# parrot-tts/Parrot-TTS

Hardware: AMD Instinct MI355X
Metric: audio samples/sec (16 kHz; see config.note) + RTF, 256-unit batch-64 per GPU (higher is better)
Workload: dtype f32 (f16x3 split products)

## Files before the change

parrot_tts_amd/csrc/conv_consts.h:

```cpp
#pragma once
namespace parrot {
enum { PRE_NONE = 0, PRE_LRELU = 1 };
enum { ACT_NONE = 0, ACT_RELU = 1, ACT_TANH = 2 };
enum { EPI_STORE = 0, EPI_ADD = 1, EPI_ADD_DIV = 2 };

constexpr int NUM_TILE_CFGS = 7;
}
```

parrot_tts_amd/csrc/host_conv.hip:

```cpp
#include "host_common.h"

#include <algorithm>
#include <cstdio>
#include <cstring>
#include <vector>

#include "conv_split.h"
#include "conv_split16.h"
#include "conv_mfma16.h"
#include "conv_valu.h"
#include "kernels_conv.h"
#include "weight_pack.h"

using namespace parrot;
static_assert(SchBf16x6::ID == PARROT_PREC_BF16X6 && SchF16x3::ID == PARROT_PREC_F16X3 && SchBf16::ID == PARROT_PREC_BF16 && SchF16::ID == PARROT_PREC_F16,
              "weight_pack.h reads a scheme off its PARROT_PREC_* number");

static int choose_cfg(int M, int k) {
    if (M <= 16) return 6;
    if (M <= 32) return 2;
    if (M <= 64) return 1;
    return (k <= 3) ? 3 : 0;
}

// ... 5 lines not shown
    static const bool on = [] { const char* e = getenv("PARROT_MFMA16"); return !e || atoi(e) != 0; }();
    return on;
}
static int small_tiles_mode() {
    static const int m = [] { const char* e = getenv("PARROT_SMALL_TILES"); return e ? atoi(e) : 2; }();
    return m;
}

int parrot::conv_build(parrot_conv** out, const parrot_conv_desc* d, int groups, const float* w, const float* bias, bool allow16) {
    if (!out || !d || !w) return fail(PARROT_E_INVALID, "conv_create: null argument");
    if (d->c_in <= 0 || d->c_out <= 0 || d->k <= 0 || d->dilation <= 0 || groups <= 0 || d->c_in % groups || d->c_out % groups)
        return fail(PARROT_E_INVALID, "conv_create: bad dimensions");
    std::unique_ptr<parrot_conv> c(new parrot_conv());
    c->d = *d;
    c->groups = groups;
    c->Cout = d->c_out;
    c->Cin = d->c_in / groups;
    int dmin = 0;
    if (d->transposed) {
        if (d->stride > 64) return fail(PARROT_E_UNSUPPORTED, "conv_create: transposed stride > 64");
        if (groups != 1 || d->dilation != 1 || d->stride <= 0) return fail(PARROT_E_UNSUPPORTED, "conv_create: transposed conv needs groups=1, dilation=1");
        const int u = d->stride, p = d->padding, k = d->k;
        int dlo = 1 << 30, dhi = -(1 << 30);
        for (int r = 0; r < u; ++r)
            for (int kap = 0; kap < k; ++kap)
                if ((r + p - kap) % u == 0) {
                    int dl = (r + p - kap) / u;
                    dlo = std::min(dlo, dl);
                    dhi = std::max(dhi, dl);
                }
        if (dlo > dhi) return fail(PARROT_E_INVALID, "conv_create: transposed conv has no taps");
        dmin = dlo;
        c->u = u;
        c->kk = dhi - dlo + 1;
        c->dil = 1;
        c->pad_left = -dlo;
        c->M = d->c_out * u;
    } else {
        if (d->stride > 1) return fail(PARROT_E_UNSUPPORTED, "conv_create: strided Conv1d is not on the path");
        c->u = 1;
        c->kk = d->k;
        c->dil = d->dilation;
        c->pad_left = d->padding;
        c->M = d->c_out;
    }
    c->Mg = c->M / groups;
    if ((c->kk - 1) * c->dil > CONV_HALO) return fail(PARROT_E_UNSUPPORTED, "conv_create: (k-1)*dilation exceeds the LDS halo (64)");
    c->cfg = (d->tile_cfg >= 0) ? d->tile_cfg : choose_cfg(c->Mg, c->kk);
    if (c->cfg >= NUM_TILE_CFGS) return fail(PARROT_E_INVALID, "conv_create: tile_cfg out of range");
    if (c->cfg == 6 && (d->transposed || groups != 1 || c->M > 16)) {
        if (d->tile_cfg == 6) return fail(PARROT_E_UNSUPPORTED, "conv_create: the 16-row tile needs a plain conv with <= 16 output channels");
        c->cfg = 2;
    }
    const TileCfg t = tile_cfg(c->cfg);
    if (groups > 1 && c->Mg % t.bm) return fail(PARROT_E_UNSUPPORTED, "conv_create: rows per group must be a multiple of the tile height");
    const int CI = t.ci, QN = CI / 8;
    c->nchunks = (c->Cin + CI - 1) / CI;
    c->n_it = c->cfg == 6 ? c->nchunks * c->kk : c->nchunks * c->kk * QN;
    const int kk = c->kk;
    const GemmWeights W{w, c->M, c->Cin, d->k, d->transposed != 0, d->c_out, c->u, d->padding, dmin};
    const int want_prec = (d->precision >= 0) ? d->precision : create_prec();
    if (want_prec > PARROT_PREC_F16) return fail(PARROT_E_INVALID, "conv_create: unknown precision");
    const bool slope_ok = d->pre_act != PRE_LRELU || (d->pre_slope >= 0.f && d->pre_slope <= 1.f);
    if (want_prec >= 1 && c->Mg >= 32 && d->tile_cfg < 0 && c->Cin % 16 == 0 && slope_ok) {
        c->prec = want_prec;
        c->cfg = (c->Mg <= 32) ? 2 : (c->Mg <= 64) ? 1 : 0;
        const TileCfg t16 = tile_cfg(c->cfg);
        if (groups > 1 && c->Mg % t16.bm) return fail(PARROT_E_UNSUPPORTED, "conv_create: rows per group must be a multiple of the tile height");
        if (scheme_is_f16(want_prec)) c->wscale = f16_weight_scale(w, (size_t)d->c_in / groups * d->c_out * d->k);
        c->mfma16 = allow16 && mfma16_enabled() && split16_has(want_prec, c->kk) && !d->transposed && groups == 1 && c->Cin % 32 == 0 && c->M >= 64;
        int rows = 32, bm = t16.bm;
        if (c->mfma16) {
            int bn16;
            rows = 16;
            split16_tile(c->M >= 128 ? 0 : 1, bm, bn16);
        }
        const int chans = 512 / rows;
        c->nchunks = (c->Cin + chans - 1) / chans;
        c->n_it16 = c->nchunks * c->kk;
        const size_t n_steps = (size_t)((c->M + bm - 1) / bm * (bm / rows)) * c->n_it16;
        const size_t n16 = (n_steps + 1) * scheme_pieces(want_prec) * 512;
        if (n16 * sizeof(uint16_t) >= ((size_t)1 << 31)) return fail(PARROT_E_UNSUPPORTED, "conv_create: packed weight stream larger than 2 GiB");
        std::vector<uint16_t> pk16(n16, 0);
        const int n_it16 = c->n_it16;
        pack_pieces(pk16.data(), n_steps, want_prec, c->wscale, W, [=](size_t st, int lane, int e) {
            const int mt = (int)(st / n_it16), ch = (int)(st % n_it16) / kk, j = (int)(st % n_it16) % kk;
            return WeightAt{mt * rows + lane % rows, ch * chans + 8 * (lane / rows) + e, j};
        });
        HIP_TRY(hipMalloc((void**)&c->wfrag16, pk16.size() * sizeof(uint16_t)));
        HIP_TRY(hipMemcpy(c->wfrag16, pk16.data(), pk16.size() * sizeof(uint16_t), hipMemcpyHostToDevice));
    } else {
        const size_t n_steps = c->cfg == 6 ? (size_t)c->n_it : (size_t)((c->M + t.bm - 1) / t.bm * (t.bm / 32)) * c->n_it;
        std::vector<float> pk((n_steps + 1) * 256, 0.f);
        if (c->cfg == 6)
            pack_f32(pk.data(), n_steps, W, [=](size_t st, int lane, int e) { return WeightAt{lane & 15, (int)st / kk * 16 + 4 * e + (lane >> 4), (int)st % kk}; });
        else {
            const int n_it = c->n_it;
            pack_f32(pk.data(), n_steps, W, [=](size_t st, int lane, int e) {
                const int mt = (int)(st / n_it), r = (int)(st % n_it), q = r % QN, j = r / QN % kk, ch = r / QN / kk;
                return WeightAt{mt * 32 + (lane & 31), ch * CI + 8 * q + 2 * e + (lane >> 5), j};
            });
        }
        HIP_TRY(hipMalloc((void**)&c->wfrag, pk.size() * sizeof(float)));
        HIP_TRY(hipMemcpy(c->wfrag, pk.data(), pk.size() * sizeof(float), hipMemcpyHostToDevice));
    }
    if (d->tile_cfg < 0 && groups == 1 && slope_ok && d->dilation == 1 && valu_kernels_enabled()) {
        if (!d->transposed && d->c_out == 1 && ((d->k == 7 && d->padding == 3) || (d->k == 1 && d->padding == 0)) &&
            (d->act == ACT_NONE || d->act == ACT_TANH))
            c->valu_kind = 1;
        if (d->transposed && d->c_out == 16 && d->k == 4 && d->stride == 2 && d->padding == 1 && d->act == ACT_NONE) c->valu_kind = 2;
        if (c->valu_kind) {
            const size_t n = (size_t)d->c_in * d->c_out * d->k;
            HIP_TRY(hipMalloc((void**)&c->wraw, n * sizeof(float)));
            HIP_TRY(hipMemcpy(c->wraw, w, n * sizeof(float), hipMemcpyHostToDevice));
        }
    }
    if (bias) {
        HIP_TRY(hipMalloc((void**)&c->bias, (size_t)d->c_out * sizeof(float)));
        HIP_TRY(hipMemcpy(c->bias, bias, (size_t)d->c_out * sizeof(float), hipMemcpyHostToDevice));
    }
    *out = c.release();
    return PARROT_OK;
}

int parrot::conv_launch(const parrot_conv* c, const float* x, const float* res, float* y, int B, int Tin, int epi, float div, hipStream_t s,
                        const ConvOpts& o) {
    const PlaneArgs& pl = o.planes;
    if (B <= 0 || Tin <= 0) return fail(PARROT_E_INVALID, "conv_run: empty batch or sequence");
    const int Tout = c->out_len(Tin);
    if (Tout <= 0) return fail(PARROT_E_INVALID, "conv_run: sequence shorter than the kernel");
    if (c->valu_kind && !res && epi == EPI_STORE && (double)c->d.c_in * Tin * 4.0 < 2147483648.0) {
        ConvValuParams q{};
        q.x = x; q.w = c->wraw; q.bias = c->bias; q.y = y;
        q.B = B; q.Cin = c->d.c_in; q.Tin = Tin; q.Tout = Tout;
        q.slope = c->d.pre_act == PRE_LRELU ? c->d.pre_slope : 1.f;
        q.act = c->d.act;
        q.row_len = o.rows.len; q.row_len_mul = o.rows.mul; q.row_len_add = o.rows.add;
        q.err = c->err_flag;
        ProfRec rec{};
        const double macs = (double)B * c->d.c_out * c->d.c_in * c->d.k * (c->d.transposed ? (double)Tin : (double)Tout);
        if (prof_on()) TRY(prof_open(rec, c->valu_kind == 1 ? PROF_VALU_CONV1 : PROF_VALU_CONVT, 2.0 * macs, 4.0 * B * ((double)c->d.c_in * Tin + (double)c->d.c_out * Tout), s));
        if (c->valu_kind == 1 && c->d.k == 7 && (Tin & 3) == 0 && (reinterpret_cast<size_t>(x) & 15) == 0 && (reinterpret_cast<size_t>(y) & 15) == 0)
            hipLaunchKernelGGL(conv1_valu7_vec_kernel, dim3((Tout + 1023) / 1024, B), dim3(256), 0, s, q);
        else if (c->valu_kind == 1 && c->d.k == 7) hipLaunchKernelGGL(conv1_valu_kernel<7>, dim3((Tout + 1023) / 1024, B), dim3(256), 0, s, q);
        else if (c->valu_kind == 1) hipLaunchKernelGGL(linear1_valu_kernel, dim3((Tout + 63) / 64, B), dim3(256), 0, s, q);
        else hipLaunchKernelGGL((convt_valu_kernel<16, 4, 2, 1>), dim3((Tin + 255) / 256, B), dim3(256), 0, s, q);
        HIP_TRY(hipGetLastError());
        if (prof_on()) TRY(prof_close(rec, s));
        return PARROT_OK;
    }
    ConvParams p{};
    p.x = x; p.wfrag = c->wfrag; p.bias = c->bias; p.res = res; p.y = y;
    p.B = B; p.Cin = c->Cin; p.Tin = Tin; p.M = c->M; p.Cout = c->Cout;
    p.Ncols = (c->u > 1) ? (Tout + c->u - 1) / c->u : Tout;
    p.Tout = Tout;
    p.k = c->kk; p.dil = c->dil; p.pad_left = c->pad_left;
    p.nchunks = c->nchunks; p.n_it = c->n_it;
    p.pre = c->d.pre_act; p.pre_slope = c->d.pre_slope; p.act = c->d.act;
    p.epi = epi; p.div = div; p.u = c->u; p.u_inv16 = (65536 + c->u - 1) / c->u;
    p.groups = c->groups; p.Mg = c->Mg;
    p.row_len = o.rows.len; p.row_len_mul = o.rows.mul; p.row_len_add = o.rows.add;
    p.acc_scale = p.out_scale = 1.f;
    p.lean = 1;
    p.n_cus = num_cus();
    p.fold_res = c->late_res ? 0 : 1;
    if (pl.xplane || pl.yplane) {
        if (!plane_ok(c) || (pl.yplane && epi != EPI_STORE)) return fail(PARROT_E_INVALID, "conv_run: operand planes need a conv_split16 layer (k = 7 / 11) and EPI_STORE");
        p.xplane = pl.xplane; p.yplane = pl.yplane;
        p.xplane_bstride = (long)plane_row_bytes(c->prec, c->Cin, Tin);
        p.yplane_bstride = (long)plane_row_bytes(c->prec, c->M, Tout);
        p.yplane_slope = pl.yslope; p.plane_only = pl.plane_only;
// ... 108 lines not shown
```

parrot_tts_amd/csrc/parrot_hip.hip:

```cpp
#include "host_common.h"

#include <algorithm>
#include <cstring>
#include <mutex>
#include <vector>

#include "conv_split.h"
#include "conv_split16.h"
#include "kernels_voc.h"
#include "resblock_split.h"
#include "resblock_fused.h"
#include "weight_pack.h"

using namespace parrot;

struct parrot_voc {
    parrot_voc_cfg cfg{};
    float* dict = nullptr;
    float* spkr = nullptr;
    DevFlag err;
    std::unique_ptr<parrot_conv> conv_pre, conv_post;
    std::vector<std::unique_ptr<parrot_conv>> ups, rb;
    std::vector<uint16_t*> rb_stream;
    std::vector<float> rb_wsc;
// ... 95 lines not shown
    const int per_rb = v->per_rb();
    if (w->n_rb != cfg->n_stages * cfg->n_kernels * per_rb) return fail(PARROT_E_INVALID, "voc_create: wrong number of resblock convs");
    query_device();
    v->scheme = create_prec();
    v->fused = create_fused();
    for (int i = 0; i < cfg->n_stages; ++i) HIP_TRY(hipEventCreateWithFlags(&v->ev_stage[i], hipEventDisableTiming));
    {
        const char* e = getenv("PARROT_PLANES");
        v->planes = e ? atoi(e) != 0 : (v->scheme == PARROT_PREC_BF16 || v->scheme == PARROT_PREC_F16);
    }
    {
        const char* e = getenv("PARROT_MRF_STREAMS");
        const bool on = e ? atoi(e) > 1 : true;
        v->mrf_auto = (e == nullptr);
        v->mrf_streams = (on && cfg->n_kernels > 1) ? cfg->n_kernels : 1;
        if (v->mrf_streams > 1) {
            for (int j = 1; j < v->mrf_streams; ++j) HIP_TRY(hipStreamCreateWithFlags(&v->ss.side[j], hipStreamNonBlocking));
            HIP_TRY(hipEventCreateWithFlags(&v->ss.ev_fork, hipEventDisableTiming));
            for (int j = 0; j < v->mrf_streams; ++j) HIP_TRY(hipEventCreateWithFlags(&v->ss.ev_last[j], hipEventDisableTiming));
        }
        for (int l = 1; l < parrot_voc::MAX_LANES; ++l) {
            HIP_TRY(hipStreamCreateWithFlags(&v->lane_stream[l], hipStreamNonBlocking));
            HIP_TRY(hipEventCreateWithFlags(&v->ev_lane_join[l], hipEventDisableTiming));
        }
        HIP_TRY(hipEventCreateWithFlags(&v->ev_lane_fork, hipEventDisableTiming));
    }
    for (int i = 0; i < cfg->n_stages; ++i) {
        const int u = cfg->upsample_rates[i], k = cfg->upsample_kernel_sizes[i];
        if (u <= 0 || k < u) return fail(PARROT_E_UNSUPPORTED, "voc_create: upsample_kernel_size must be >= upsample_rate (negative padding)");
        if ((k - u) & 1) v->odd_stage = true;
    }
    TRY(upload(&v->dict, w->dict, (size_t)cfg->num_embeddings * cfg->embedding_dim));
    if (cfg->multispkr) {
        if (!w->spkr) return fail(PARROT_E_INVALID, "voc_create: multispkr without spkr table");
        TRY(upload(&v->spkr, w->spkr, (size_t)cfg->n_spkr * cfg->embedding_dim));
    }
    TRY(v->err.init());
    const int C0 = cfg->upsample_initial_channel;
    TRY(make_conv(v->conv_pre, cfg->model_in_dim, C0, 7, 1, 3, 0, 1, PRE_NONE, 0.f, ACT_NONE, w->conv_pre_w, w->conv_pre_b));
    v->ups.resize(cfg->n_stages);
    v->rb.resize(w->n_rb);
    for (int i = 0; i < cfg->n_stages; ++i) {
        const int cin = C0 >> i, cout = C0 >> (i + 1), u = cfg->upsample_rates[i], k = cfg->upsample_kernel_sizes[i];
        v->up_total *= u;
        TRY(make_conv(v->ups[i], cin, cout, k, 1, (k - u) / 2, 1, u, PRE_LRELU, 0.1f, ACT_NONE, w->ups_w[i], w->ups_b[i]));
        for (int j = 0; j < cfg->n_kernels; ++j) {
            const int rk = cfg->resblock_kernel_sizes[j];
            const bool a16 = !(v->fused != 0 && cfg->resblock_type == 1 && resblock_split_has(cout, rk) && per_rb <= RBS_MAX_CONVS);
            for (int m = 0; m < cfg->n_dil; ++m) {
                const int dl = cfg->resblock_dilation_sizes[j][m];
                const int base = v->rb_base(i, j);
                if (cfg->resblock_type == 1) {
                    TRY(make_conv(v->rb[base + 2 * m], cout, cout, rk, dl, (rk * dl - dl) / 2, 0, 1, PRE_LRELU, 0.1f, ACT_NONE,
                                  w->rb_w[base + 2 * m], w->rb_b[base + 2 * m], 1, a16));
                    TRY(make_conv(v->rb[base + 2 * m + 1], cout, cout, rk, 1, (rk - 1) / 2, 0, 1, PRE_LRELU, 0.1f, ACT_NONE,
                                  w->rb_w[base + 2 * m + 1], w->rb_b[base + 2 * m + 1], 1, a16));
                } else {
                    TRY(make_conv(v->rb[base + m], cout, cout, rk, dl, (rk * dl - dl) / 2, 0, 1, PRE_LRELU, 0.1f, ACT_NONE,
                                  w->rb_w[base + m], w->rb_b[base + m], 1, a16));
                }
            }
        }
    }
    v->rb_stream.assign((size_t)cfg->n_stages * cfg->n_kernels, nullptr);
    v->rb_wsc.assign((size_t)w->n_rb, 1.f);
    v->rb_conv_halves.assign((size_t)cfg->n_stages * cfg->n_kernels, 0);
    const int NP = scheme_pieces(v->scheme);
    for (int i = 0; i < cfg->n_stages && v->scheme >= 1; ++i)
        for (int j = 0; j < cfg->n_kernels; ++j) {
            const int rk = cfg->resblock_kernel_sizes[j], C = v->chan(i);
            if (cfg->resblock_type != 1 || !resblock_split_has(C, rk) || per_rb > RBS_MAX_CONVS) continue;
            const int base = v->rb_base(i, j);
            const int steps = resblock_split_steps(C, rk);
            const size_t step_b = (size_t)NP * 1024, conv_b = (size_t)steps * step_b;
            v->rb_conv_halves[v->branch(i, j)] = conv_b / 2;
            if (C >= 32) {
                bool ok = true;
                for (int q = 0; q < per_rb; ++q) {
                    const parrot_conv* pc = v->rb[base + q].get();
                    ok = ok && pc->prec == v->scheme && !pc->mfma16 && pc->wfrag16 && pc->nchunks == C / 16 && (C / 32) * pc->n_it16 == steps && pc->M == C &&
                         C % tile_cfg(pc->cfg).bm == 0;
                }
                if (!ok) continue;
                uint16_t* st = nullptr;
                HIP_TRY(hipMalloc((void**)&st, (per_rb + 1) * conv_b));
                v->rb_stream[v->branch(i, j)] = st;
                for (int q = 0; q <= per_rb; ++q)
                    HIP_TRY(hipMemcpy(reinterpret_cast<char*>(st) + q * conv_b, v->rb[base + (q < per_rb ? q : 0)]->wfrag16, conv_b, hipMemcpyDeviceToDevice));
                for (int q = 0; q < per_rb; ++q) v->rb_wsc[base + q] = v->rb[base + q]->wscale;
            } else {
                const size_t step_h = (size_t)NP * 512;
                std::vector<uint16_t> pk(((size_t)per_rb * steps + 2) * step_h, 0);
                for (int q = 0; q < per_rb; ++q) {
                    const GemmWeights W{w->rb_w[base + q], 16, 16, rk, false, 0, 1, 0, 0};
                    const float wsc = scheme_is_f16(v->scheme) ? f16_weight_scale(W.w, (size_t)16 * 16 * rk) : 1.f;
                    v->rb_wsc[base + q] = wsc;
                    pack_pieces(pk.data() + (size_t)q * steps * step_h, steps, v->scheme, wsc, W, [](size_t st, int lane, int e) {
                        return WeightAt{lane & 15, 8 * ((lane >> 4) & 1) + e, 2 * (int)st + (lane >> 5)};
                    });
                }
                uint16_t* st = nullptr;
                HIP_TRY(hipMalloc((void**)&st, pk.size() * sizeof(uint16_t)));
                v->rb_stream[v->branch(i, j)] = st;
                HIP_TRY(hipMemcpy(st, pk.data(), pk.size() * sizeof(uint16_t), hipMemcpyHostToDevice));
            }
        }
    v->mrf_ok.assign((size_t)cfg->n_stages, 0);
    {
        static const bool want = [] { const char* e = getenv("PARROT_MRF_FUSED"); return !e || atoi(e) != 0; }();
        for (int i = 0; i < cfg->n_stages && want && v->fused != 0 && v->scheme >= 1 && resblock_mrf_scheme(v->scheme); ++i) {
            const int C = v->chan(i);
            if (cfg->resblock_type != 1 || !resblock_mrf_has(C) || per_rb > RBS_MAX_CONVS || cfg->n_kernels > RBS_MAX_BRANCH) continue;
            bool ok = true;
            for (int j = 0; j < cfg->n_kernels; ++j) ok = ok && (cfg->resblock_kernel_sizes[j] & 1) && v->branch_stream(i, j);
            v->mrf_ok[i] = ok && rbs_mrf_window(C) - 2 * v->stage_reach(i) >= rbs_mrf_window(C) / 2;
        }
    }
    TRY(make_conv(v->conv_post, C0 >> cfg->n_stages, 1, 7, 1, 3, 0, 1, PRE_LRELU, 0.01f, ACT_TANH, w->conv_post_w, w->conv_post_b));
    v->conv_post->err_flag = v->err;
    *out = v.release();
    return PARROT_OK;
}
extern "C" int parrot_voc_create(parrot_voc_t** out, const parrot_voc_cfg* cfg, const parrot_voc_weights* w) { return voc_create(out, cfg, w, -1, -1); }
extern "C" int parrot_voc_create_ex(parrot_voc_t** out, const parrot_voc_cfg* cfg, const parrot_voc_weights* w, int32_t precision,
                                    int32_t fused_resblocks) {
    if (precision > PARROT_PREC_F16 || fused_resblocks > 2) return fail(PARROT_E_INVALID, "voc_create_ex: precision in -1 .. 4, fused_resblocks in -1 .. 2");
    return voc_create(out, cfg, w, precision, fused_resblocks);
}
extern "C" void parrot_voc_destroy(parrot_voc_t* v) { delete v; }
extern "C" int parrot_voc_precision(const parrot_voc_t* v) { return v ? v->scheme : PARROT_E_INVALID; }
extern "C" int parrot_voc_debug_absmax(parrot_voc_t* v, float* dst_dev) {
    if (!v) return fail(PARROT_E_INVALID, "voc_debug_absmax: null handle");
    v->dbg_absmax = dst_dev;
    return PARROT_OK;
}

static size_t voc_max_act(const parrot_voc* v, int B, int U) {
    size_t mx = (size_t)B * v->cfg.upsample_initial_channel * U;
    int T = U;
    for (int i = 0; i < v->cfg.n_stages; ++i) {
        T = v->ups[i]->out_len(T);
        mx = std::max(mx, (size_t)B * v->chan(i) * (size_t)T);
    }
    return mx;
}
static long voc_out_len(const parrot_voc* v, int U) {
    long T = U;
    for (int i = 0; i < v->cfg.n_stages; ++i) T = v->ups[i]->out_len((int)T);
    return T;
}
extern "C" int64_t parrot_voc_out_len(const parrot_voc_t* v, int32_t U) { return (v && U > 0) ? voc_out_len(v, U) : 0; }

static bool resblock_fusable(const parrot_voc* v, int stage, int j) {
    const parrot_voc_cfg& c = v->cfg;
    const int C = v->chan(stage), k = c.resblock_kernel_sizes[j];
    const int fm = v->fused;
    if (fm == 0 || !(C == 16 || (C == 32 && fm == 1)) || !(k & 1)) return false;
    const int per_rb = v->per_rb(), base = v->rb_base(stage, j);
    if (per_rb > RB_MAX_CONVS) return false;
    for (int m = 0; m < c.n_dil; ++m)
        if ((k - 1) / 2 * c.resblock_dilation_sizes[j][m] > RB_PAD) return false;
    for (int q = 0; q < per_rb; ++q)
        if (v->rb[base + q]->prec != 0 || v->rb[base + q]->cfg != (C == 16 ? 6 : 2) || !v->rb[base + q]->wfrag) return false;
    return resblock_window(C) - 2 * v->branch_reach(stage, j) >= 128;
}
struct Branch {
    const float* x;
    float* y;
    float *mid, *res_a, *res_b;
    int B, T, epi;
    float div;
// ... 566 lines not shown
```

parrot_tts_amd/csrc/resblock_split.h:

```cpp
#pragma once
#include "conv_split.h"

namespace parrot {

constexpr int RBS_MAX_CONVS = 8;
constexpr int RBS_MAX_BRANCH = 4;
constexpr int RBS_MAX_ALL = RBS_MAX_CONVS * RBS_MAX_BRANCH;

#ifdef RBS_TRACE
constexpr int RBS_TRACE_STAMPS = 128;
__device__ unsigned long long g_rbs_trace[8 * RBS_TRACE_STAMPS];
#define RBS_STAMP()                                                                                                   \
    do {                                                                                                              \
        if (trace_on && trace_n < RBS_TRACE_STAMPS) {                                                                 \
            const unsigned long long tt = __builtin_amdgcn_s_memtime();                                               \
            if (lane == 0) g_rbs_trace[wave * RBS_TRACE_STAMPS + trace_n] = tt;                                       \
        }                                                                                                             \
        ++trace_n;                                                                                                    \
    } while (0)
#else
#define RBS_STAMP() do {} while (0)
#endif
#ifndef RBS_EARLY_INNER
#define RBS_EARLY_INNER 1
#endif

struct ResblockSplitParams {
    const float* x;
    float* y;
    const uint16_t* wstream;
    const float* bias[RBS_MAX_ALL];
    float wsc[RBS_MAX_ALL];
    int dil[RBS_MAX_ALL];
    int n_conv;
    int k;
    int early;
    int n_branch;
    const uint16_t* bstream[RBS_MAX_BRANCH];
    int bk[RBS_MAX_BRANCH];
    int T, B;
    int H;
    int TT;
    int tiles;
    int epi;
    float div;
    float slope;
    const int32_t* row_len;
    int row_len_mul;
    int row_len_add;
};

constexpr int RBS_W = 384;

constexpr int rbs_default_wn(int nch) { return (nch / 2 >= 4) ? 1 : 4 / (nch / 2); }
template <class SCH, int NCH, int WN = 0, bool MRF = false>
__global__ __launch_bounds__((NCH / 2) * (WN ? WN : rbs_default_wn(NCH)) * 64,
                             ((NCH / 2) * (WN ? WN : rbs_default_wn(NCH)) * 64 == 512) ? 1 : (SCH::NP == 3 ? 2 : 3)) void resblock_split_kernel(const ResblockSplitParams p) {
    constexpr int NPC = SCH::NP, NTERM = SCH::NT, STEP_BYTES = SCH::NP * 1024;
    constexpr int C = 16 * NCH, WAVES_M = NCH / 2, WAVES_N = WN ? WN : rbs_default_wn(NCH), NTW = 3, W = WAVES_N * NTW * 32;
    const bool early = (WAVES_M == 1) && RBS_EARLY_INNER && __builtin_amdgcn_readfirstlane(p.early) != 0;
    int K = MRF ? p.bk[0] : p.k;
    constexpr int OCT_BYTES = W * 16, CH_BYTES = 2 * OCT_BYTES, PIECE_BYTES = NCH * CH_BYTES;
    static_assert(NCH == 2 || NCH == 4 || NCH == 8 || NCH == 16, "32, 64, 128 channels (4 waves: NCH / 2 row tiles x 4 / (NCH / 2) column groups) or 256 (8 waves)");
    extern __shared__ __attribute__((aligned(16))) char smem_raw[];

    const int tid = threadIdx.x;
    const int lane = tid & 63;
    const int wave = __builtin_amdgcn_readfirstlane(tid >> 6);
    const int wm = wave / WAVES_N;
    const int wn = wave % WAVES_N;
    const int half = lane >> 5;
    const int l31 = lane & 31;
    const int b = blockIdx.x / p.tiles;
    const int tile = blockIdx.x - b * p.tiles;
    const int t_base = tile * p.TT - p.H;
    const int Tlim = p.row_len ? min(p.T, row_true_len(p.row_len[b], p.row_len_mul, p.row_len_add)) : p.T;
    const bool edge = __builtin_amdgcn_readfirstlane((t_base < 0 || t_base + W > Tlim) ? 1 : 0);
#ifdef RBS_TRACE
    const bool trace_on = NCH == 2 && blockIdx.x == gridDim.x / 2;
    int trace_n = 0;
    RBS_STAMP();
#endif

    int col[NTW];
    bool tok[NTW];
#pragma unroll
    for (int nt = 0; nt < NTW; ++nt) {
        col[nt] = wn * (NTW * 32) + nt * 32 + l31;
        const int t = t_base + col[nt];
        tok[nt] = t >= 0 && t < Tlim;
    }

    f32x16 R[NTW], acc[NTW];
    auto load_r = [&]() __attribute__((always_inline)) {
        const size_t xaddr = reinterpret_cast<size_t>(p.x + (size_t)b * C * p.T);
        const unsigned x_lo = __builtin_amdgcn_readfirstlane((unsigned)xaddr), x_hi = __builtin_amdgcn_readfirstlane((unsigned)(xaddr >> 32));
        const __amdgpu_buffer_rsrc_t xrsrc =
            __builtin_amdgcn_make_buffer_rsrc(reinterpret_cast<void*>(((size_t)x_hi << 32) | x_lo), 0, 0x7fffffff, 0x00020000);
        const int row_bytes = p.T * 4;
#pragma unroll
        for (int nt = 0; nt < NTW; ++nt) {
            const int voff = tok[nt] ? (t_base + col[nt]) * 4 + 4 * half * row_bytes : (int)0x80000000;
#pragma unroll
            for (int r = 0; r < 16; ++r)
                R[nt][r] = __builtin_bit_cast(float, __builtin_amdgcn_raw_buffer_load_b32(xrsrc, voff, (32 * wm + (r & 3) + 8 * (r >> 2)) * row_bytes, 0));
        }
    };
    load_r();

    auto write_p = [&](const f32x16 (&v)[NTW], float mul, int part = 0) __attribute__((always_inline)) {
#pragma unroll
        for (int nt = 0; nt < NTW; ++nt) {
            if (part != 0 && (nt == 1) != (part == 1)) continue;
            const float m2 = (SCH::XS != 1.f) ? mul * p.slope : p.slope;
#pragma unroll
            for (int q = 0; q < 2; ++q) {
                unsigned qq[2][2][NPC];
#pragma unroll
                for (int g = 0; g < 2; ++g)
#pragma unroll
                    for (int e = 0; e < 2; ++e) {
                        const f32x2 vv = {v[nt][8 * q + 4 * g + 2 * e], v[nt][8 * q + 4 * g + 2 * e + 1]};
                        const f32x2 a = (SCH::XS != 1.f) ? vv * mul : vv, bq = vv * m2;
                        SCH::split(max_nc(a[0], bq[0]), max_nc(a[1], bq[1]), qq[g][e]);
                    }
                char* dst = smem_raw + (2 * wm + q) * CH_BYTES + half * OCT_BYTES + col[nt] * 16;
#pragma unroll
                for (int pc = 0; pc < NPC; ++pc) {
                    const auto r0 = __builtin_amdgcn_permlane32_swap(qq[0][0][pc], qq[1][0][pc], false, false);
                    const auto r1 = __builtin_amdgcn_permlane32_swap(qq[0][1][pc], qq[1][1][pc], false, false);
                    *reinterpret_cast<uint4*>(dst + pc * PIECE_BYTES) = uint4{r0[0], r1[0], r0[1], r1[1]};
                }
            }
        }
        if (edge) {
#pragma unroll
            for (int nt = 0; nt < NTW; ++nt)
                if (!tok[nt] && (part == 0 || (nt == 1) == (part == 1))) {
#pragma unroll
                    for (int q = 0; q < 2; ++q)
#pragma unroll
                        for (int pc = 0; pc < NPC; ++pc)
                            *reinterpret_cast<uint4*>(smem_raw + (2 * wm + q) * CH_BYTES + half * OCT_BYTES + col[nt] * 16 + pc * PIECE_BYTES) = uint4{0u, 0u, 0u, 0u};
                }
        }
    };

    auto stream_rsrc = [&](const uint16_t* ws) __attribute__((always_inline)) {
        const unsigned w_lo = __builtin_amdgcn_readfirstlane((unsigned)reinterpret_cast<size_t>(ws));
        const unsigned w_hi = __builtin_amdgcn_readfirstlane((unsigned)(reinterpret_cast<size_t>(ws) >> 32));
        return __builtin_amdgcn_make_buffer_rsrc(reinterpret_cast<void*>(((size_t)w_hi << 32) | w_lo), 0, 0x7fffffff, 0x00020000);
    };
    __amdgpu_buffer_rsrc_t wrsrc = stream_rsrc(MRF ? p.bstream[0] : p.wstream);
    const unsigned lane16 = lane * 16;
    s16x8 A[2][NPC], Bv[2][NTW][NPC];
    auto load_a_piece = [&](s16x8 (&a)[NPC], int pc, int gstep) __attribute__((always_inline)) {
        a[pc] = __builtin_bit_cast(s16x8, __builtin_amdgcn_raw_buffer_load_b128(wrsrc, lane16 + pc * 1024, gstep * STEP_BYTES, 0));
    };
    int conv_steps = WAVES_M * NCH * K;
    int gbase = wm * NCH * K;
#pragma unroll
    for (int pc = 0; pc < NPC; ++pc) {
        load_a_piece(A[0], pc, gbase);
        load_a_piece(A[1], pc, gbase + K);
    }

    RBS_STAMP();
    write_p(R, SCH::XS);
    RBS_STAMP();
    __syncthreads();
    RBS_STAMP();

    int center = (K - 1) / 2;
    auto load_b = [&](s16x8 (&bb)[NTW][NPC], int ch, int shift) __attribute__((always_inline)) {
#pragma unroll
        for (int nt = 0; nt < NTW; ++nt) {
            const char* src = smem_raw + ch * CH_BYTES + half * OCT_BYTES + (col[nt] + shift) * 16;
#pragma unroll
            for (int pc = 0; pc < NPC; ++pc) bb[nt][pc] = *reinterpret_cast<const s16x8*>(src + pc * PIECE_BYTES);
        }
    };
    auto conv = [&](f32x16 (&acc)[NTW], int dil) __attribute__((always_inline)) {
        load_b(Bv[0], 0, -center * dil);
        for (int j = 0; j < K; ++j) {
            const int shift = (j - center) * dil;
            const int n0 = (j + 1 < K) ? gbase + j + 1 : gbase + conv_steps;
#pragma unroll
            for (int ch = 0; ch < NCH; ++ch) {
                const int set = ch & 1;
                if (ch + 1 < NCH) load_b(Bv[set ^ 1], ch + 1, shift);
                else load_b(Bv[set ^ 1], 0, shift + dil);
                const int nx = (ch + 2 < NCH) ? gbase + (ch + 2) * K + j : n0 + (ch + 2 - NCH) * K;
#pragma unroll
                for (int t = 0; t < NTERM; ++t) {
#pragma unroll
                    for (int nt = 0; nt < NTW; ++nt) acc[nt] = mfma32<SCH>(A[set][SCH::pa(t)], Bv[set][nt][SCH::pb(t)], acc[nt]);
#pragma unroll
                    for (int pc = 0; pc < NPC; ++pc)
                        if (t == SCH::last_a(pc)) load_a_piece(A[set], pc, nx);
                }
            }
#pragma unroll
            for (int ch = 0; ch < NCH; ++ch) {
                int ds_left = NPC * NTW;
#pragma unroll
                for (int m = 0; m < NTERM * NTW; ++m) {
                    __builtin_amdgcn_sched_group_barrier(0x008, 1, 0);
                    bool refetch = false;
#pragma unroll
                    for (int pc = 1; pc < NPC; ++pc) refetch = refetch || (m == (SCH::last_a(pc) + 1) * NTW - 1);
                    if (refetch) __builtin_amdgcn_sched_group_barrier(0x020, 1, 0);
                    else if (ds_left > 0) {
                        __builtin_amdgcn_sched_group_barrier(0x100, 1, 0);
                        --ds_left;
                    }
                }
                __builtin_amdgcn_sched_group_barrier(0x020, 1, 0);
            }
            __builtin_amdgcn_sched_barrier(0);
        }
        gbase += conv_steps;
    };
    auto bias_rows = [&](const float* __restrict__ bias, float (&bv)[16]) __attribute__((always_inline)) {
#pragma unroll
        for (int r = 0; r < 16; ++r) bv[r] = bias[32 * wm + (r & 3) + 8 * (r >> 2) + 4 * half];
    };

    f32x16 XSr[MRF ? NTW : 1];
    const int n_branch = MRF ? p.n_branch : 1;
    for (int br = 0; br < n_branch; ++br) {
    if (MRF && br > 0) {
        K = p.bk[br];
        center = (K - 1) / 2;
        conv_steps = WAVES_M * NCH * K;
        gbase = wm * NCH * K;
        wrsrc = stream_rsrc(p.bstream[br]);
        load_r();
#pragma unroll
        for (int pc = 0; pc < NPC; ++pc) {
            load_a_piece(A[0], pc, gbase);
            load_a_piece(A[1], pc, gbase + K);
        }
        RBS_STAMP();
        __syncthreads();
        RBS_STAMP();
        write_p(R, SCH::XS);
        RBS_STAMP();
        __syncthreads();
        RBS_STAMP();
    }
    float rs = 1.f;
    for (int mm = 0; mm < p.n_conv; mm += 2) {
        const int m = br * p.n_conv + mm;
        float bv[16];
        const float s1 = SCH::XS * p.wsc[m], s2 = SCH::XS * p.wsc[m + 1];
        bias_rows(p.bias[m], bv);
#pragma unroll
        for (int nt = 0; nt < NTW; ++nt)
#pragma unroll
            for (int r = 0; r < 16; ++r) acc[nt][r] = (SCH::XS != 1.f) ? bv[r] * s1 : bv[r];
        RBS_STAMP();
        conv(acc, p.dil[m]);
        RBS_STAMP();
        if (early) write_p(acc, 1.f / p.wsc[m], 1);
        RBS_STAMP();
        __syncthreads();
        RBS_STAMP();
        write_p(acc, 1.f / p.wsc[m], early ? 2 : 0);
        RBS_STAMP();
        __syncthreads();
        RBS_STAMP();
        bias_rows(p.bias[m + 1], bv);
        if constexpr (SCH::XS != 1.f) {
            const float ratio = s2 / rs;
#pragma unroll
            for (int r = 0; r < 16; ++r) bv[r] = bv[r] * s2;
#pragma unroll
            for (int nt = 0; nt < NTW; ++nt)
#pragma unroll
                for (int r = 0; r < 16; ++r) R[nt][r] = __builtin_fmaf(R[nt][r], ratio, bv[r]);
        } else {
#pragma unroll
            for (int nt = 0; nt < NTW; ++nt)
#pragma unroll
                for (int r = 0; r < 16; ++r) R[nt][r] = bv[r] + R[nt][r];
        }
        RBS_STAMP();
        conv(R, p.dil[m + 1]);
        RBS_STAMP();
        rs = (SCH::XS != 1.f) ? s2 : 1.f;
        if (mm + 2 < p.n_conv) {
            if (early) write_p(R, SCH::XS / rs, 1);
            RBS_STAMP();
            __syncthreads();
            RBS_STAMP();
            write_p(R, SCH::XS / rs, early ? 2 : 0);
            RBS_STAMP();
            __syncthreads();
            RBS_STAMP();
        }
    }
    if constexpr (SCH::XS != 1.f) {
        const float inv = 1.f / rs;
#pragma unroll
        for (int nt = 0; nt < NTW; ++nt)
#pragma unroll
            for (int r = 0; r < 16; ++r) R[nt][r] = R[nt][r] * inv;
    }
    if constexpr (MRF) {
#pragma unroll
        for (int nt = 0; nt < NTW; ++nt)
#pragma unroll
            for (int r = 0; r < 16; ++r) XSr[nt][r] = (br == 0) ? 0.f + R[nt][r] : XSr[nt][r] + R[nt][r];
    }
    }

    RBS_STAMP();
    const RowTile yt = row_tile(p.y + (size_t)b * C * p.T, C, p.T);
    const int row_bytes = p.T * 4;
    const bool has_acc = !MRF && p.epi != EPI_STORE;
    const bool do_div = p.epi == EPI_ADD_DIV;
#pragma unroll
    for (int nt = 0; nt < NTW; ++nt) {
        const int c = col[nt] - p.H;
        const int t = tile * p.TT + c;
        const bool ok = c >= 0 && c < p.TT && t < p.T;
        const int voff = ok ? (4 * half * p.T + t) * 4 : (int)0x80000000;
        float v[16];
        if constexpr (MRF) {
#pragma unroll
            for (int r = 0; r < 16; ++r) v[r] = (n_branch > 1) ? XSr[nt][r] / p.div : XSr[nt][r];
        } else if (has_acc) {
            float yv[16];
#pragma unroll
            for (int r = 0; r < 16; ++r) yv[r] = row_tile_load(yt, voff, (32 * wm + (r & 3) + 8 * (r >> 2)) * row_bytes);
#pragma unroll
            for (int r = 0; r < 16; ++r) v[r] = yv[r] + R[nt][r];
            if (do_div) {
#pragma unroll
                for (int r = 0; r < 16; ++r) v[r] = v[r] / p.div;
            }
        } else {
#pragma unroll
            for (int r = 0; r < 16; ++r) v[r] = 0.f + R[nt][r];
        }
#pragma unroll
        for (int r = 0; r < 16; ++r) row_tile_store(yt, v[r], voff, (32 * wm + (r & 3) + 8 * (r >> 2)) * row_bytes);
    }
}

constexpr int RBS16_W = 768;

template <class SCH>
__global__ __launch_bounds__(256, SCH::NP == 3 ? 2 : 3) void resblock16_split_kernel(const ResblockSplitParams p) {
    constexpr int NPC = SCH::NP, NTERM = SCH::NT, STEP_BYTES = SCH::NP * 1024;
    constexpr int C = 16, NT = 12, W = RBS16_W, NP = NT / 2;
    const int K = p.k, S = (K + 1) / 2;
    constexpr int OCT_BYTES = W * 16, PIECE_BYTES = 2 * OCT_BYTES;
    static_assert(4 * NT * 16 == W, "4 waves x NT tiles cover the window");
    extern __shared__ __attribute__((aligned(16))) char smem_raw[];

    const int tid = threadIdx.x;
    const int lane = tid & 63;
    const int wave = __builtin_amdgcn_readfirstlane(tid >> 6);
    const int g4 = lane >> 4;
    const int l15 = lane & 15;
    const int b = blockIdx.x / p.tiles;
    const int tile = blockIdx.x - b * p.tiles;
    const int t_base = tile * p.TT - p.H;
    const int Tlim = p.row_len ? min(p.T, row_true_len(p.row_len[b], p.row_len_mul, p.row_len_add)) : p.T;
    const bool edge = __builtin_amdgcn_readfirstlane((t_base < 0 || t_base + W > Tlim) ? 1 : 0);
    const int col0 = wave * (NT * 16) + l15;
    const bool early = RBS_EARLY_INNER && __builtin_amdgcn_readfirstlane(p.early) != 0;

    f32x4 R[NT], acc[NT];
    {
        const size_t xaddr = reinterpret_cast<size_t>(p.x + (size_t)b * C * p.T);
        const unsigned x_lo = __builtin_amdgcn_readfirstlane((unsigned)xaddr), x_hi = __builtin_amdgcn_readfirstlane((unsigned)(xaddr >> 32));
        const __amdgpu_buffer_rsrc_t xrsrc =
            __builtin_amdgcn_make_buffer_rsrc(reinterpret_cast<void*>(((size_t)x_hi << 32) | x_lo), 0, 0x7fffffff, 0x00020000);
        const int row_bytes = p.T * 4;
#pragma unroll
        for (int nt = 0; nt < NT; ++nt) {
            const int t = t_base + col0 + nt * 16;
            const int voff = (t >= 0 && t < Tlim) ? t * 4 + 4 * g4 * row_bytes : (int)0x80000000;
#pragma unroll
            for (int r = 0; r < 4; ++r) R[nt][r] = __builtin_bit_cast(float, __builtin_amdgcn_raw_buffer_load_b32(xrsrc, voff, r * row_bytes, 0));
        }
    }
    auto write_p = [&](const f32x4 (&v)[NT], float mul, int part = 0) __attribute__((always_inline)) {
        const float m2 = (SCH::XS != 1.f) ? mul * p.slope : p.slope;
#pragma unroll
        for (int np = 0; np < NT; np += 2) {
            if (part != 0 && (np >= 2 && np < NT - 2) != (part == 1)) continue;
            unsigned qq[2][2][NPC];
#pragma unroll
            for (int u = 0; u < 2; ++u) {
#pragma unroll
                for (int e = 0; e < 2; ++e) {
                    const f32x2 vv = {v[np + u][2 * e], v[np + u][2 * e + 1]};
                    const f32x2 a = (SCH::XS != 1.f) ? vv * mul : vv, bq = vv * m2;
                    SCH::split(max_nc(a[0], bq[0]), max_nc(a[1], bq[1]), qq[u][e]);
                }
            }
            const int c = col0 + (np + (g4 & 1)) * 16;
            char* dst = smem_raw + (g4 >> 1) * OCT_BYTES + c * 16;
#pragma unroll
            for (int pc = 0; pc < NPC; ++pc) {
                const auto r0 = __builtin_amdgcn_permlane16_swap(qq[0][0][pc], qq[1][0][pc], false, false);
                const auto r1 = __builtin_amdgcn_permlane16_swap(qq[0][1][pc], qq[1][1][pc], false, false);
                *reinterpret_cast<uint4*>(dst + pc * PIECE_BYTES) = uint4{r0[0], r1[0], r0[1], r1[1]};
            }
        }
        if (edge) {
#pragma unroll
            for (int np = 0; np < NT; np += 2) {
                if (part != 0 && (np >= 2 && np < NT - 2) != (part == 1)) continue;
                const int c = col0 + (np + (g4 & 1)) * 16;
                const int t = t_base + c;
                if (!(t >= 0 && t < Tlim)) {
#pragma unroll
                    for (int pc = 0; pc < NPC; ++pc)
                        *reinterpret_cast<uint4*>(smem_raw + (g4 >> 1) * OCT_BYTES + c * 16 + pc * PIECE_BYTES) = uint4{0u, 0u, 0u, 0u};
                }
            }
        }
    };

    const unsigned w_lo = __builtin_amdgcn_readfirstlane((unsigned)reinterpret_cast<size_t>(p.wstream));
    const unsigned w_hi = __builtin_amdgcn_readfirstlane((unsigned)(reinterpret_cast<size_t>(p.wstream) >> 32));
// ... 205 lines not shown
```

parrot_tts_amd/csrc/weight_pack.h:

```cpp
#pragma once
#include <stdint.h>

#include <algorithm>
#include <cmath>
#include <cstring>
#include <vector>

#include "../../include/parrot_hip.h"

namespace parrot {

inline int scheme_pieces(int scheme) { return scheme == PARROT_PREC_BF16X6 ? 3 : scheme == PARROT_PREC_F16X3 ? 2 : 1; }
inline bool scheme_is_f16(int scheme) { return scheme == PARROT_PREC_F16X3 || scheme == PARROT_PREC_F16; }
inline float scheme_xs(int scheme) { return scheme_is_f16(scheme) ? 8.f : 1.f; }

inline uint16_t f16_rn_host(float x) {
    const _Float16 h = (_Float16)x;
    uint16_t u;
    memcpy(&u, &h, 2);
    return u;
}
inline float f16_to_f(uint16_t u) {
    _Float16 h;
    memcpy(&h, &u, 2);
    return (float)h;
}
inline uint16_t bf16_rn_host(float x) {
    uint32_t u;
    memcpy(&u, &x, 4);
    u += 0x7fffu + ((u >> 16) & 1u);
    return (uint16_t)(u >> 16);
}
inline float bf16_to_f(uint16_t h) {
    uint32_t u = (uint32_t)h << 16;
    float f;
    memcpy(&f, &u, 4);
    return f;
}

inline float f16_weight_scale(const float* w, size_t n) {
    float mx = 0.f;
    for (size_t i = 0; i < n; ++i) mx = std::max(mx, std::fabs(w[i]));
    if (!(mx > 0.f) || !std::isfinite(mx)) return 1.f;
    int e;
    (void)std::frexp(mx, &e);
    return std::ldexp(1.f, 15 - e);
}
inline void split_weight(float v, int scheme, float wscale, uint16_t (&h)[3]) {
    h[0] = h[1] = h[2] = 0;
    if (scheme_is_f16(scheme)) {
        const float vs = v * wscale;
        h[0] = f16_rn_host(vs);
        if (scheme == PARROT_PREC_F16X3) h[1] = f16_rn_host(vs - f16_to_f(h[0]));
        return;
    }
    h[0] = bf16_rn_host(v);
    if (scheme == PARROT_PREC_BF16X6) {
        const float r1 = v - bf16_to_f(h[0]);
        h[1] = bf16_rn_host(r1);
        h[2] = bf16_rn_host(r1 - bf16_to_f(h[1]));
    }
}

struct GemmWeights {
    const float* w;
    int M, Cin, k;
    bool transposed;
    int c_out, u, padding, dmin;
    float operator()(int m, int i, int j) const {
        if (m >= M || i >= Cin) return 0.f;
        if (transposed) {
            const int o = m / u, r = m % u;
            const int kap = r + padding - (j + dmin) * u;
            return (kap >= 0 && kap < k) ? w[((size_t)i * c_out + o) * k + kap] : 0.f;
        }
        return j < k ? w[((size_t)m * Cin + i) * k + j] : 0.f;
    }
};
struct WeightAt {
    int m, i, j;
};

struct ChainGroups { int G, Mg; };
inline ChainGroups chain_groups(int scheme, int cin, int rows) {
    int G = 1;
    if (scheme == PARROT_PREC_F32)
        for (int g = 8; g > 1 && G == 1; --g)
            if (cin % (16 * g) == 0) G = g;
    return {G, G > 1 ? (rows + 127) / 128 * 128 : rows};
}

template <typename Layout>
inline void pack_f32(float* dst, size_t n_steps, const GemmWeights& W, Layout at) {
    for (size_t st = 0; st < n_steps; ++st)
        for (int lane = 0; lane < 64; ++lane)
            for (int e = 0; e < 4; ++e) {
                const WeightAt q = at(st, lane, e);
                dst[st * 256 + lane * 4 + e] = W(q.m, q.i, q.j);
            }
}
template <typename Layout>
inline void pack_pieces(uint16_t* dst, size_t n_steps, int scheme, float wscale, const GemmWeights& W, Layout at) {
    const int NP = scheme_pieces(scheme);
    for (size_t st = 0; st < n_steps; ++st) {
        uint16_t* g = dst + st * NP * 512;
        for (int lane = 0; lane < 64; ++lane)
            for (int e = 0; e < 8; ++e) {
                const WeightAt q = at(st, lane, e);
                uint16_t h[3];
                split_weight(W(q.m, q.i, q.j), scheme, wscale, h);
                for (int pc = 0; pc < NP; ++pc) g[pc * 512 + lane * 8 + e] = h[pc];
            }
    }
}

}
```

Before: 306.4 million.

## Relabel resblock weight rows to drop permlane32 swaps in LDS staging

Applies a fixed row permutation (swapping bits 2 and 3 of the row index) to the packed resblock weight stream on the host. The kernel's row addressing for loads, bias and stores is changed to match. Because of this relabelling, the per-piece permlane32_swap shuffles before the LDS store can be dropped and the registers written directly. It adds host-side repacking instead of a device copy, and depends on every row index site staying consistent with the permutation.

```diff
diff --git a/parrot_tts_amd/csrc/conv_consts.h b/parrot_tts_amd/csrc/conv_consts.h
--- a/parrot_tts_amd/csrc/conv_consts.h
+++ b/parrot_tts_amd/csrc/conv_consts.h
@@ -5,4 +5,12 @@
 enum { EPI_STORE = 0, EPI_ADD = 1, EPI_ADD_DIV = 2 };
 
 constexpr int NUM_TILE_CFGS = 7;
+
+constexpr int rbs_row_sigma(int m) { return (m & ~12) | ((m & 4) << 1) | ((m & 8) >> 1); }
+constexpr bool rbs_row_sigma_is_involution() {
+    for (int m = 0; m < 32; ++m)
+        if (rbs_row_sigma(m) < 0 || rbs_row_sigma(m) >= 32 || rbs_row_sigma(rbs_row_sigma(m)) != m) return false;
+    return true;
 }
+static_assert(rbs_row_sigma_is_involution(), "rbs_row_sigma: an involution on the rows 0..31 of a tile");
+}
diff --git a/parrot_tts_amd/csrc/host_conv.hip b/parrot_tts_amd/csrc/host_conv.hip
--- a/parrot_tts_amd/csrc/host_conv.hip
+++ b/parrot_tts_amd/csrc/host_conv.hip
@@ -111,11 +111,7 @@
         const size_t n16 = (n_steps + 1) * scheme_pieces(want_prec) * 512;
         if (n16 * sizeof(uint16_t) >= ((size_t)1 << 31)) return fail(PARROT_E_UNSUPPORTED, "conv_create: packed weight stream larger than 2 GiB");
         std::vector<uint16_t> pk16(n16, 0);
-        const int n_it16 = c->n_it16;
-        pack_pieces(pk16.data(), n_steps, want_prec, c->wscale, W, [=](size_t st, int lane, int e) {
-            const int mt = (int)(st / n_it16), ch = (int)(st % n_it16) / kk, j = (int)(st % n_it16) % kk;
-            return WeightAt{mt * rows + lane % rows, ch * chans + 8 * (lane / rows) + e, j};
-        });
+        pack_pieces(pk16.data(), n_steps, want_prec, c->wscale, W, TileStreamLayout{rows, c->n_it16, kk, false});
         HIP_TRY(hipMalloc((void**)&c->wfrag16, pk16.size() * sizeof(uint16_t)));
         HIP_TRY(hipMemcpy(c->wfrag16, pk16.data(), pk16.size() * sizeof(uint16_t), hipMemcpyHostToDevice));
     } else {
diff --git a/parrot_tts_amd/csrc/parrot_hip.hip b/parrot_tts_amd/csrc/parrot_hip.hip
--- a/parrot_tts_amd/csrc/parrot_hip.hip
+++ b/parrot_tts_amd/csrc/parrot_hip.hip
@@ -201,11 +201,17 @@
                          C % tile_cfg(pc->cfg).bm == 0;
                 }
                 if (!ok) continue;
+                const size_t conv_h = conv_b / 2;
+                std::vector<uint16_t> pk((size_t)(per_rb + 1) * conv_h, 0);
+                for (int q = 0; q <= per_rb; ++q) {
+                    const parrot_conv* pc = v->rb[base + (q < per_rb ? q : 0)].get();
+                    const GemmWeights W{w->rb_w[base + (q < per_rb ? q : 0)], C, C, rk, false, 0, 1, 0, 0};
+                    pack_pieces(pk.data() + q * conv_h, steps, v->scheme, pc->wscale, W, TileStreamLayout{32, pc->n_it16, rk, true});
+                }
                 uint16_t* st = nullptr;
-                HIP_TRY(hipMalloc((void**)&st, (per_rb + 1) * conv_b));
+                HIP_TRY(hipMalloc((void**)&st, pk.size() * sizeof(uint16_t)));
                 v->rb_stream[v->branch(i, j)] = st;
-                for (int q = 0; q <= per_rb; ++q)
-                    HIP_TRY(hipMemcpy(reinterpret_cast<char*>(st) + q * conv_b, v->rb[base + (q < per_rb ? q : 0)]->wfrag16, conv_b, hipMemcpyDeviceToDevice));
+                HIP_TRY(hipMemcpy(st, pk.data(), pk.size() * sizeof(uint16_t), hipMemcpyHostToDevice));
                 for (int q = 0; q < per_rb; ++q) v->rb_wsc[base + q] = v->rb[base + q]->wscale;
             } else {
                 const size_t step_h = (size_t)NP * 512;
diff --git a/parrot_tts_amd/csrc/resblock_split.h b/parrot_tts_amd/csrc/resblock_split.h
--- a/parrot_tts_amd/csrc/resblock_split.h
+++ b/parrot_tts_amd/csrc/resblock_split.h
@@ -91,6 +91,8 @@
         tok[nt] = t >= 0 && t < Tlim;
     }
 
+    auto row_of = [&](int r) __attribute__((always_inline)) { return 32 * wm + rbs_row_sigma((r & 3) + 8 * (r >> 2)); };
+    static_assert(rbs_row_sigma(4) == 8 && rbs_row_sigma(3 + 8 * 3) == 16 + 4 + 3, "half h of a lane adds sigma(4 h) = 8 h channels");
     f32x16 R[NTW], acc[NTW];
     auto load_r = [&]() __attribute__((always_inline)) {
         const size_t xaddr = reinterpret_cast<size_t>(p.x + (size_t)b * C * p.T);
@@ -100,10 +102,10 @@
         const int row_bytes = p.T * 4;
 #pragma unroll
         for (int nt = 0; nt < NTW; ++nt) {
-            const int voff = tok[nt] ? (t_base + col[nt]) * 4 + 4 * half * row_bytes : (int)0x80000000;
+            const int voff = tok[nt] ? (t_base + col[nt]) * 4 + 8 * half * row_bytes : (int)0x80000000;
 #pragma unroll
             for (int r = 0; r < 16; ++r)
-                R[nt][r] = __builtin_bit_cast(float, __builtin_amdgcn_raw_buffer_load_b32(xrsrc, voff, (32 * wm + (r & 3) + 8 * (r >> 2)) * row_bytes, 0));
+                R[nt][r] = __builtin_bit_cast(float, __builtin_amdgcn_raw_buffer_load_b32(xrsrc, voff, row_of(r) * row_bytes, 0));
         }
     };
     load_r();
@@ -126,11 +128,8 @@
                     }
                 char* dst = smem_raw + (2 * wm + q) * CH_BYTES + half * OCT_BYTES + col[nt] * 16;
 #pragma unroll
-                for (int pc = 0; pc < NPC; ++pc) {
-                    const auto r0 = __builtin_amdgcn_permlane32_swap(qq[0][0][pc], qq[1][0][pc], false, false);
-                    const auto r1 = __builtin_amdgcn_permlane32_swap(qq[0][1][pc], qq[1][1][pc], false, false);
-                    *reinterpret_cast<uint4*>(dst + pc * PIECE_BYTES) = uint4{r0[0], r1[0], r0[1], r1[1]};
-                }
+                for (int pc = 0; pc < NPC; ++pc)
+                    *reinterpret_cast<uint4*>(dst + pc * PIECE_BYTES) = uint4{qq[0][0][pc], qq[0][1][pc], qq[1][0][pc], qq[1][1][pc]};
             }
         }
         if (edge) {
@@ -223,7 +222,7 @@
     };
     auto bias_rows = [&](const float* __restrict__ bias, float (&bv)[16]) __attribute__((always_inline)) {
 #pragma unroll
-        for (int r = 0; r < 16; ++r) bv[r] = bias[32 * wm + (r & 3) + 8 * (r >> 2) + 4 * half];
+        for (int r = 0; r < 16; ++r) bv[r] = bias[row_of(r) + 8 * half];
     };
 
     f32x16 XSr[MRF ? NTW : 1];
@@ -325,7 +324,7 @@
         const int c = col[nt] - p.H;
         const int t = tile * p.TT + c;
         const bool ok = c >= 0 && c < p.TT && t < p.T;
-        const int voff = ok ? (4 * half * p.T + t) * 4 : (int)0x80000000;
+        const int voff = ok ? (8 * half * p.T + t) * 4 : (int)0x80000000;
         float v[16];
         if constexpr (MRF) {
 #pragma unroll
@@ -333,7 +332,7 @@
         } else if (has_acc) {
             float yv[16];
 #pragma unroll
-            for (int r = 0; r < 16; ++r) yv[r] = row_tile_load(yt, voff, (32 * wm + (r & 3) + 8 * (r >> 2)) * row_bytes);
+            for (int r = 0; r < 16; ++r) yv[r] = row_tile_load(yt, voff, row_of(r) * row_bytes);
 #pragma unroll
             for (int r = 0; r < 16; ++r) v[r] = yv[r] + R[nt][r];
             if (do_div) {
@@ -345,7 +344,7 @@
             for (int r = 0; r < 16; ++r) v[r] = 0.f + R[nt][r];
         }
 #pragma unroll
-        for (int r = 0; r < 16; ++r) row_tile_store(yt, v[r], voff, (32 * wm + (r & 3) + 8 * (r >> 2)) * row_bytes);
+        for (int r = 0; r < 16; ++r) row_tile_store(yt, v[r], voff, row_of(r) * row_bytes);
     }
 }
 
diff --git a/parrot_tts_amd/csrc/weight_pack.h b/parrot_tts_amd/csrc/weight_pack.h
--- a/parrot_tts_amd/csrc/weight_pack.h
+++ b/parrot_tts_amd/csrc/weight_pack.h
@@ -7,6 +7,7 @@
 #include <vector>
 
 #include "../../include/parrot_hip.h"
+#include "conv_consts.h"
 
 namespace parrot {
 
@@ -80,6 +81,15 @@
 struct WeightAt {
     int m, i, j;
 };
+struct TileStreamLayout {
+    int rows, n_it, k;
+    bool relabel;
+    WeightAt operator()(size_t st, int lane, int e) const {
+        const int mt = (int)(st / n_it), ch = (int)(st % n_it) / k, j = (int)(st % n_it) % k;
+        const int row = relabel ? rbs_row_sigma(lane % rows) : lane % rows;
+        return WeightAt{mt * rows + row, ch * (512 / rows) + 8 * (lane / rows) + e, j};
+    }
+};
 
 struct ChainGroups { int G, Mg; };
 inline ChainGroups chain_groups(int scheme, int cin, int rows) {
```

Result: no change. 307.6 million, median of 6 (+0.4%).
